# sydeng99/ssTEM-restoration

Hardware: AMD Instinct MI355X
Metric: restored megapixels/sec (interp+fusion fwd) at 1024x1024; PSNR vs ref (higher is better)
Workload: dtype f32; 1 GPU; SepConv 51-tap interpolation forward (pad + 2 sepconv + add + mean; one fused launch on the two gray planes, row-segment coefficients as the IFNet heads store them), batch=8 1024x1024 tiles per GPU; batch_per_gpu=8, taps=51, frame_planes=1, coefficient_layout=row-segments, compare_with_rounds_1_2=extra.apply_nchw_1024

## Files before the change

### sstem-restoration_amd/csrc/sepconv_kernels.hip

```cpp
#include <hip/hip_runtime.h>
#include <stdint.h>
#include <stdlib.h>

#include <atomic>
#include <mutex>
#include <unordered_map>

#include "sepconv_kernels.h"

#ifndef SSTEM_ABLATE
#define SSTEM_ABLATE 0
#endif
#ifndef SSTEM_HPF
#define SSTEM_HPF 11
#endif
#ifndef SSTEM_BLK_SKEWLD
#define SSTEM_BLK_SKEWLD 0
#endif
#ifndef SSTEM_GRAY_DMA
#define SSTEM_GRAY_DMA 1
#endif
#ifndef SSTEM_RGB_RING
#define SSTEM_RGB_RING 2
#endif
#ifndef SSTEM_GRAY16_ABLATE
#define SSTEM_GRAY16_ABLATE 0
#endif
#ifndef SSTEM_COEF_AUX
#define SSTEM_COEF_AUX 0
#endif
#ifndef SSTEM_PAIR_COEF_AUX
#define SSTEM_PAIR_COEF_AUX 2
#endif

namespace sstem {

constexpr int F = 51;
constexpr int KSTEPS = 54;
constexpr int TILE_COLS = 116;

__host__ __device__ constexpr int rm_pitch(int ch) { return ch == 2 ? 120 : 144; }
__host__ __device__ constexpr int rm_pitch_tile(int ch, int waves, int rpw)
{
    return (waves * rpw > 36) ? TILE_COLS : rm_pitch(ch);
}
static_assert((1 * rm_pitch(1) / 4) % 16 == 4 && (2 * rm_pitch(2) / 4) % 16 == 12 &&
              (3 * rm_pitch(3) / 4) % 16 == 12 && rm_pitch(2) >= TILE_COLS, "LDS row stride");

typedef float f32x4 __attribute__((ext_vector_type(4)));

template <bool BF> __device__ __forceinline__ float coef_at(const float* t, int64_t i)
{
    if constexpr (BF) return __builtin_bit_cast(float, (uint32_t)reinterpret_cast<const uint16_t*>(t)[i] << 16);
    else return t[i];
}
template <bool BF = false>
__global__ __launch_bounds__(256) void sepconv_fwd_direct(
    const float* __restrict__ in, const float* __restrict__ ver, const float* __restrict__ hor,
    float* __restrict__ out, int64_t B, int64_t C, int64_t H, int64_t W, int filt, const int* __restrict__ skip_if_gray = nullptr)
{
    if (skip_if_gray && *skip_if_gray != 0) return;
    const int64_t plane = H * W;
    const int64_t Hin = H + filt - 1, Win = W + filt - 1;
    const int64_t n = B * plane;
    for (int64_t p = (int64_t)blockIdx.x * blockDim.x + threadIdx.x; p < n;
         p += (int64_t)gridDim.x * blockDim.x) {
        const int64_t b = p / plane;
        const int64_t yx = p - b * plane;
        const int64_t y = yx / W, x = yx - y * W;
        const int64_t cbase = b * filt * plane + yx;
        for (int64_t c = 0; c < C; ++c) {
            const float* ip = in + ((b * C + c) * Hin + y) * Win + x;
            float acc = 0.f;
            for (int fy = 0; fy < filt; ++fy) {
                float t = 0.f;
                for (int fx = 0; fx < filt; ++fx)
                    t = fmaf(ip[(int64_t)fy * Win + fx], coef_at<BF>(hor, cbase + (int64_t)fx * plane), t);
                acc = fmaf(coef_at<BF>(ver, cbase + (int64_t)fy * plane), t, acc);
            }
            out[(b * C + c) * plane + yx] = acc;
        }
    }
}

template <bool VERTICAL, bool BF = false>
__global__ __launch_bounds__(256) void sepconv_grad_direct(
    const float* __restrict__ g, const float* __restrict__ in, const float* __restrict__ coef,
    float* __restrict__ gout, int64_t B, int64_t C, int64_t H, int64_t W, int filt, const int* __restrict__ skip_if_gray = nullptr)
{
    if (skip_if_gray && *skip_if_gray != 0) return;
    const int64_t plane = H * W;
    const int64_t Hin = H + filt - 1, Win = W + filt - 1;
    const int64_t n = B * filt * plane;
    for (int64_t p = (int64_t)blockIdx.x * blockDim.x + threadIdx.x; p < n;
         p += (int64_t)gridDim.x * blockDim.x) {
        const int64_t b = p / (filt * plane);
        const int64_t r = p - b * filt * plane;
        const int64_t f = r / plane;
        const int64_t yx = r - f * plane;
        const int64_t y = yx / W, x = yx - y * W;
        const int64_t cbase = b * filt * plane + yx;
        float acc = 0.f;
        for (int64_t c = 0; c < C; ++c) {
            const float gg = g[(b * C + c) * plane + yx];
            const float* ip = in + ((b * C + c) * Hin + y) * Win + x;
            float t = 0.f;
            if (VERTICAL) {
                for (int fx = 0; fx < filt; ++fx)
                    t = fmaf(ip[f * Win + fx], coef_at<BF>(coef, cbase + (int64_t)fx * plane), t);
            } else {
                for (int fy = 0; fy < filt; ++fy)
                    t = fmaf(ip[(int64_t)fy * Win + f], coef_at<BF>(coef, cbase + (int64_t)fy * plane), t);
            }
            acc = fmaf(gg, t, acc);
        }
        gout[p] = acc;
    }
}
// ... 785 lines not shown
                    const float res = ph ? (parked + csum) * (1.0f / 3) : csum;
                    *stg_ptr(dst, xoff) = res;
                    if (ph && fa.out_u8) fa.out_u8[(b * H + y) * W + x0 + lane] = numpy_u8_of(res);
                }
            }
            if constexpr (!PFH && BLK && SSTEM_BLK_SKEWLD) load_taps_skewed_buf(hc, rh, nextoff, pn, xoff, sub);
            else if constexpr (!PFH) load_taps_buf<BF>(hc, rh, nextoff, pn, xoff);
        };
        int nrows = 0;
        if (y0 + ywave < H) {
            const int64_t left = (H - 1 - (y0 + ywave)) / YSTEP + 1;
            nrows = left < RPW ? (int)left : RPW;
        }
        if constexpr (PFH) {
#pragma unroll 1
            for (int rr = 0; rr + 1 < nrows; rr += 2) {
                do_row(hs, hn, rr, true);
                do_row(hn, hs, rr + 1, rr + 2 < nrows);
            }
            if (nrows & 1) {
                do_row(hs, hn, nrows - 1, false);
                if (next_ph) {
#pragma unroll
                    for (int t = 0; t < KSTEPS; ++t) hs[t] = hn[t];
                }
            }
        } else {
            float dummy[1];
#pragma unroll 1
            for (int rr = 0; rr < nrows; ++rr) do_row(hs, dummy, rr, rr + 1 < nrows);
        }
    }
}

template <int I, int N, typename Fn>
__device__ __forceinline__ void static_for(Fn&& fn)
{
    if constexpr (I < N) {
        fn(std::integral_constant<int, I>{});
        static_for<I + 1, N>(fn);
    }
}

template <int WAVES, int RPW, int WPE>
__global__ __launch_bounds__(WAVES * 64, WPE) void sepconv_gray_mfma_pair(
    const float* __restrict__ in_a, const float* __restrict__ ver_a, const float* __restrict__ hor_a,
    float* __restrict__ out, TileArgs args, FusedArgs fa)
{
    static_assert(WAVES == 4, "the rows of a pair are one 4-row MFMA tile apart");
    static_assert(RPW % 2 == 0, "row pairs");
    if (fa.gray_flag && *fa.gray_flag == 0) return;
    constexpr int TR = WAVES * RPW;
    constexpr int ROWS = TR + F;
    constexpr int RS = rm_pitch(1);
    constexpr int YSTEP = WAVES;
    constexpr int NA = 2;
    constexpr int NGRP = 7;
    constexpr int LV = 2;
    constexpr uint32_t TAP = 256u;
    constexpr int AUX = SSTEM_PAIR_COEF_AUX;
    extern __shared__ __attribute__((aligned(16))) float lds[];

    int64_t b, ty, tx;
    decode_block(args, b, ty, tx);
    const int64_t H = args.H, W = args.W;
    const int64_t plane = H * W;
    const int wave = __builtin_amdgcn_readfirstlane(threadIdx.x >> 6);
    const int64_t y0 = ty * TR, x0 = tx * 64;

    const int lane = threadIdx.x & 63;
    const int blk = lane >> 2, sub = lane & 3;
    const bool xok = (x0 + lane) < W;
    const uint32_t xoff = (uint32_t)(xok ? lane : 0) * 4u;
    auto clampy = [&](int64_t y) __attribute__((always_inline)) -> int64_t { return y < H ? y : H - 1; };
    const int64_t yfirst = clampy(y0 + wave);

    const uint32_t seg_row = (uint32_t)args.tiles_x * (uint32_t)(F * 256);
    const uint32_t img_bytes = (uint32_t)H * seg_row;
    const int64_t img_elems = (int64_t)(img_bytes >> 2);
    const uint32_t seg_x = (uint32_t)tx * (uint32_t)(F * 256);
    auto rowoff = [&](int64_t y) __attribute__((always_inline)) -> uint32_t { return (uint32_t)clampy(y) * seg_row + seg_x; };

    float hA[KSTEPS], hB[KSTEPS], vA[F], vB[F];

    auto vload = [&](float (&v)[F], rsrc_t r, uint32_t ro, uint32_t ps, const int f0, const int f1) __attribute__((always_inline)) {
        uint32_t soff = ro + (uint32_t)f0 * ps;
        pin_s(soff);
#pragma unroll
        for (int f = 0; f < F; ++f) {
            if (f < f0 || f >= f1) continue;
            v[f] = bldc<false, AUX>(r, xoff, soff);
            soff += ps;
            pin_s(soff);
        }
    };
    auto vload_group = [&](const int k, rsrc_t r, uint32_t roA, uint32_t roB, uint32_t ps) __attribute__((always_inline)) {
        vload(vA, r, roA, ps, 8 * k, (8 * k + 8 < F) ? 8 * k + 8 : F);
        vload(vB, r, roB, ps, (8 * k - 4 > 0) ? 8 * k - 4 : 0, (8 * k + 4 < F) ? 8 * k + 4 : F);
    };
    auto hload = [&](float (&h)[KSTEPS], rsrc_t r, uint32_t ro, uint32_t ps, const int t0, const int t1) __attribute__((always_inline)) {
        if constexpr (SSTEM_BLK_SKEWLD) load_taps_skewed_buf<AUX>(h, r, ro, ps, xoff, sub, t0, t1 < KSTEPS ? t1 : KSTEPS);
        else load_taps_buf<false, AUX>(h, r, ro, ps, xoff, t0 < F ? t0 : F, t1 < F ? t1 : F);
    };
    {
        const rsrc_t rv = coef_rsrc_c<false>(ver_a, b * img_elems, img_bytes);
        const rsrc_t rh = coef_rsrc_c<false>(hor_a, b * img_elems, img_bytes);
        const uint32_t oA = rowoff(yfirst), oB = rowoff(yfirst + YSTEP);
#pragma unroll
        for (int k = 0; k < LV; ++k) vload_group(k, rv, oA, oB, TAP);
        hload(hA, rh, oA, TAP, 0, KSTEPS);
        hload(hB, rh, oB, TAP, 0, KSTEPS);
    }

#pragma unroll 1
    for (int ph = 0; ph < 2; ++ph) {
        const float* in = ph ? fa.in2 : in_a;
        const float* ver = ph ? fa.ver2 : ver_a;
        const float* hor = ph ? fa.hor2 : hor_a;
        const bool next_ph = ph == 0;
        const rsrc_t rv_cur = coef_rsrc_c<false>(ver, b * img_elems, img_bytes);
        const rsrc_t rh_cur = coef_rsrc_c<false>(hor, b * img_elems, img_bytes);
        const rsrc_t rv_nxt = coef_rsrc_c<false>(next_ph ? fa.ver2 : ver, b * img_elems, img_bytes);
        const rsrc_t rh_nxt = coef_rsrc_c<false>(next_ph ? fa.hor2 : hor, b * img_elems, img_bytes);

        if (ph) __syncthreads();
#if SSTEM_GRAY_DMA
        stage_gray_tile_dma<WAVES * 64, ROWS, RS, true>(lds, in + (b * args.in_planes) * plane, (int)H, (int)W, (int)y0, (int)x0);
#else
        stage_gray_tile<WAVES * 64, ROWS, RS, true>(lds, in + (b * args.in_planes) * plane, (int)H, (int)W, (int)y0, (int)x0);
#endif
        __syncthreads();

        int nrows = 0;
        if (y0 + wave < H) {
            const int64_t left = (H - 1 - (y0 + wave)) / YSTEP + 1;
            nrows = left < RPW ? (int)left : RPW;
        }
#pragma unroll 1
        for (int rr = 0; rr < nrows; rr += 2) {
            const bool more = rr + 2 < nrows;
            const bool two = rr + 1 < nrows;
            const int yl = wave + rr * YSTEP;
            const int64_t y = y0 + yl;
            const int64_t ynext = more ? (y + 2 * YSTEP) : (next_ph ? yfirst : y);
            const uint32_t pn = (more || next_ph) ? TAP : 0u;
            const uint32_t curA = rowoff(y), curB = rowoff(y + YSTEP);
            const uint32_t nxtA = rowoff(ynext), nxtB = rowoff(ynext + YSTEP);
            const rsrc_t rv_n = more ? rv_cur : rv_nxt;
            const rsrc_t rh_n = more ? rh_cur : rh_nxt;
            float* dstA = out + (b * H + y) * W + x0;
            float* dstB = out + (b * H + clampy(y + YSTEP)) * W + x0;
            pin_uniform(dstA);
            pin_uniform(dstB);
            const float parkedA = *stg_ptr(dstA, xoff);
            const float parkedB = *stg_ptr(dstB, xoff);

            if constexpr (!SSTEM_BLK_SKEWLD) {
                skew_taps_in_place(hA, sub);
                skew_taps_in_place(hB, sub);
            }
            const float* arow = lds + (yl + sub) * RS + blk * 4;
            f32x4 ar[2][NA];
#pragma unroll
            for (int c = 0; c < NA; ++c) ar[0][c] = *reinterpret_cast<const f32x4*>(arow + c * 4 * RS);
            float oA = 0.f, oB = 0.f;
            static_for<0, NGRP>([&](auto kc) __attribute__((always_inline)) {
                constexpr int k = decltype(kc)::value;
                if (k + LV < NGRP) vload_group(k + LV, rv_cur, curA, curB, TAP);
                else vload_group(k + LV - NGRP, rv_n, nxtA, nxtB, pn);
                f32x4 accA[NA], accB[NA];
#pragma unroll
                for (int c = 0; c < NA; ++c) { accA[c] = (f32x4){0.f, 0.f, 0.f, 0.f}; accB[c] = accA[c]; }
                const float* abase = arow + k * (NA * 4) * RS;
                const float* anext = arow + (k + 1) * (NA * 4) * RS;
#pragma unroll
                for (int tq = 0; tq < 14; ++tq) {
                    const int cc = k * 14 + tq;
                    if (tq + 1 < 14) {
#pragma unroll
                        for (int c = 0; c < NA; ++c)
                            ar[(cc + 1) % 2][c] = *reinterpret_cast<const f32x4*>(abase + c * 4 * RS + (tq + 1) * 4);
                    } else if (k + 1 < NGRP) {
#pragma unroll
                        for (int c = 0; c < NA; ++c)
                            ar[(cc + 1) % 2][c] = *reinterpret_cast<const f32x4*>(anext + c * 4 * RS);
                    }
                    __builtin_amdgcn_sched_barrier(0);
#pragma unroll
                    for (int e = 0; e < 4; ++e) {
                        const int t = tq * 4 + e;
                        if (t < KSTEPS) {
#pragma unroll
                            for (int c = 0; c < NA; ++c) {
                                const int a = 2 * k + c;
                                if (a <= 12) accA[c] = __builtin_amdgcn_mfma_f32_4x4x1f32(ar[cc % 2][c][e], hA[t], accA[c], 0, 0, 0);
                                if (a >= 1) accB[c] = __builtin_amdgcn_mfma_f32_4x4x1f32(ar[cc % 2][c][e], hB[t], accB[c], 0, 0, 0);
                            }
                        }
                    }
                    __builtin_amdgcn_sched_barrier(0);
                    if (k == NGRP - 1) {
                        hload(hA, rh_n, nxtA, pn, 4 * tq, 4 * tq + 4);
                        hload(hB, rh_n, nxtB, pn, 4 * tq, 4 * tq + 4);
                    }
                }
#pragma unroll
                for (int c = 0; c < NA; ++c) {
                    const int a = 2 * k + c;
                    if (a <= 12)
#pragma unroll
                        for (int i = 0; i < 4; ++i)
                            if (4 * a + i < F) oA = fmaf(vA[4 * a + i], accA[c][i], oA);
                }
#pragma unroll
                for (int c = 0; c < NA; ++c) {
                    const int a = 2 * k + c;
                    if (a >= 1)
#pragma unroll
                        for (int i = 0; i < 4; ++i)
                            if (4 * (a - 1) + i < F) oB = fmaf(vB[4 * (a - 1) + i], accB[c][i], oB);
                }
                asm volatile("" : "+v"(oA), "+v"(oB));
            });
            if (xok) {
                const float csA = (oA + oA) + oA;
                const float resA = ph ? (parkedA + csA) * (1.0f / 3) : csA;
                *stg_ptr(dstA, xoff) = resA;
                if (ph && fa.out_u8) fa.out_u8[(b * H + y) * W + x0 + lane] = numpy_u8_of(resA);
                if (two) {
                    const float csB = (oB + oB) + oB;
                    const float resB = ph ? (parkedB + csB) * (1.0f / 3) : csB;
                    *stg_ptr(dstB, xoff) = resB;
                    if (ph && fa.out_u8) fa.out_u8[(b * H + y + YSTEP) * W + x0 + lane] = numpy_u8_of(resB);
                }
            }
        }
    }
}

constexpr int G16_RS = 130;
template <int WAVES, int RPW, bool BLK, int VAR = 0>
__global__ __launch_bounds__(WAVES * 64, 2) void sepconv_gray16_mfma(
    const float* __restrict__ in_a, const float* __restrict__ ver_a, const float* __restrict__ hor_a,
    float* __restrict__ out, TileArgs args, FusedArgs fa)
{
    constexpr int TR = WAVES * RPW;
    constexpr int ROWS = TR + F;
    constexpr int RS = G16_RS;
    constexpr int IMG = ROWS * RS;
    extern __shared__ __attribute__((aligned(16))) float lds[];

    int64_t b, ty, tx;
    decode_block(args, b, ty, tx);
    const int64_t H = args.H, W = args.W;
    const int64_t plane = H * W;
    const int wave = __builtin_amdgcn_readfirstlane(threadIdx.x >> 6);
    const int64_t y0 = ty * TR, x0 = tx * 64;
    const int lane = threadIdx.x & 63;
    const int kq = lane >> 4, j = lane & 15;

    const uint32_t tap4 = BLK ? 256u : (uint32_t)plane * 4u;
    const uint32_t seg_row = (uint32_t)args.tiles_x * (uint32_t)(F * 256);
    const uint32_t img_bytes = BLK ? (uint32_t)H * seg_row : (uint32_t)F * tap4;
    const int64_t img_elems = BLK ? (int64_t)(img_bytes >> 2) : (int64_t)F * plane;
    const uint32_t seg_x = (uint32_t)tx * (uint32_t)(F * 256);
    auto rowoff = [&](int64_t y) __attribute__((always_inline)) -> uint32_t {
        return BLK ? (uint32_t)y * seg_row + seg_x : (uint32_t)(y * W + x0) * 4u;
    };
    const rsrc_t rv0 = coef_rsrc(ver_a + b * img_elems, img_bytes), rh0 = coef_rsrc(hor_a + b * img_elems, img_bytes);
    const rsrc_t rv1 = coef_rsrc(fa.ver2 + b * img_elems, img_bytes), rh1 = coef_rsrc(fa.hor2 + b * img_elems, img_bytes);

    const int d = kq - j;
    const int c = d & 3, sh = -(d >> 2);
    const bool s1 = sh & 1, s2 = sh & 2, s4 = sh & 4, c3 = c == 3;
    const uint32_t vh = (uint32_t)c * tap4 + (uint32_t)j * 4u;
    const uint32_t vv = (uint32_t)(4 * kq) * tap4 + (uint32_t)j * 4u;
    const uint32_t vr = (uint32_t)j * 4u;

    float Bh[4][17], Vv[4][15];
    auto request = [&](const int cg0, const int NC, const rsrc_t rh, const rsrc_t rv, const uint32_t off) __attribute__((always_inline)) {
        uint32_t so = off;
        pin_s(so);
#pragma unroll
        for (int n = 0; n < 13; ++n) {
#pragma unroll
            for (int q = 0; q < NC; ++q) Bh[cg0 + q][n] = bld(rh, vh + (uint32_t)(cg0 + q) * 64u, so);
            so += 4u * tap4;
            pin_s(so);
        }
#pragma unroll
        for (int T = 0; T < 3; ++T) {
            so = off + (uint32_t)(16 * T) * tap4;
            pin_s(so);
#pragma unroll
            for (int r = 0; r < 4; ++r) {
#pragma unroll
                for (int q = 0; q < NC; ++q) Vv[cg0 + q][4 * T + r] = bld(rv, vv + (uint32_t)(cg0 + q) * 64u, so);
                so += tap4;
                pin_s(so);
            }
        }
        so = off + 48u * tap4;
        pin_s(so);
#pragma unroll
        for (int r = 0; r < 3; ++r) {
#pragma unroll
            for (int q = 0; q < NC; ++q) Vv[cg0 + q][12 + r] = bld(rv, vr + (uint32_t)(cg0 + q) * 64u, so);
            so += tap4;
            pin_s(so);
        }
    };

    int nrows = 0;
    if (y0 + wave < H) {
        const int64_t left = (H - 1 - (y0 + wave)) / WAVES + 1;
        nrows = left < RPW ? (int)left : RPW;
    }
    if (nrows > 0) {
        const uint32_t off = rowoff(y0 + wave);
        request(0, 2, rh0, rv0, off);
// ... 1339 lines not shown
                                 const TileArgs& a, hipStream_t s, const int* flag = nullptr)
{
    return gradh_coalesce() ? launch_gradh_vc<CH, WAVES, RPW, true>(in, g, ver, gh, a, s, flag)
                            : launch_gradh_vc<CH, WAVES, RPW, false>(in, g, ver, gh, a, s, flag);
}

static hipError_t launch_rgb_gradh_stream(const float* in, const float* g, const float* ver, float* gh, TileArgs a, hipStream_t s,
                                          const int* flag)
{
    constexpr int WAVES = 8, RPW = 4, TR = WAVES * RPW;
    constexpr int ROWS = TR + F + 4;
    constexpr int PITCH_T = ((ROWS + 3) / 4 * 4) | 4;
    constexpr size_t lds_bytes = (size_t)3 * TCOLS * PITCH_T * sizeof(float);
    static_assert(lds_bytes <= 160 * 1024, "LDS");
    auto k = sepconv_rgb_gradh_stream_mfma<WAVES, RPW>;
    static std::atomic<uint64_t> lds_set{0};
    const hipError_t attr = set_lds(k, lds_bytes, lds_set);
    if (attr != hipSuccess) return attr;
    a.tiles_y = (a.H + TR - 1) / TR;
    const int64_t nwg = a.B * a.tiles_y * a.tiles_x;
    if (nwg <= 0 || nwg > 0x7fffffffLL) return hipErrorInvalidValue;
    hipLaunchKernelGGL(k, dim3((unsigned)nwg), dim3(WAVES * 64), lds_bytes, s, in, g, ver, gh, a, flag);
    return hipGetLastError();
}

template <int CH>
static hipError_t launch_gradh(const float* in, const float* g, const float* ver, float* gh,
                               const TileArgs& a, hipStream_t s)
{
    switch (tile_variant()) {
        case 1: return launch_gradh_v<CH, 12, 3>(in, g, ver, gh, a, s);
        case 2: return launch_gradh_v<CH, 12, 2>(in, g, ver, gh, a, s);
        case 3: return launch_gradh_v<CH, 16, 2>(in, g, ver, gh, a, s);
        case 4: return launch_gradh_v<CH, 16, 3>(in, g, ver, gh, a, s);
        default: return launch_gradh_v<CH, 8, 4>(in, g, ver, gh, a, s);
    }
}

static TileArgs make_args(int64_t B, int64_t C, int64_t H, int64_t W)
{
    TileArgs a;
    a.B = B; a.C = C; a.H = H; a.W = W;
    a.tiles_x = (W + 63) / 64;
    const int tr = tile_rows(tile_variant());
    a.tiles_y = (H + tr - 1) / tr;
    a.c0 = 0;
    a.in_planes = 3;
    static const int dbg = [] { const char* d = getenv("SSTEM_DEBUG_FLAGS"); return d ? atoi(d) : 0; }();
    a.dbg = dbg;
    return a;
}

bool mfma_grid_ok(int64_t B, int64_t H, int64_t W)
{
    TileArgs a = make_args(B, 1, H, W);
    const int64_t nwg = a.B * a.tiles_y * a.tiles_x;
    return nwg > 0 && nwg <= 0x7fffffffLL;
}

template <int MODE, int WAVES, int RPW, int WPE, bool PFH, int RING, bool BLK = false, bool BF = false>
static hipError_t launch_gray_v(const float* in, const float* ver, const float* hor, float* out, TileArgs a,
                                hipStream_t s, const FusedArgs& fa)
{
    constexpr int TR = WAVES * RPW;
    constexpr size_t lds_bytes = (size_t)(TR + F) * rm_pitch(1) * sizeof(float);
    static_assert(lds_bytes <= 160 * 1024, "LDS");
    auto k = sepconv_gray_mfma<MODE, WAVES, RPW, WPE, PFH, RING, BLK, BF>;
    static std::atomic<uint64_t> lds_set{0};
    const hipError_t attr = set_lds(k, lds_bytes, lds_set);
    if (attr != hipSuccess) return attr;
    a.tiles_y = (a.H + TR - 1) / TR;
    const int64_t nwg = a.B * a.tiles_y * a.tiles_x;
    if (nwg <= 0 || nwg > 0x7fffffffLL) return hipErrorInvalidValue;
    hipLaunchKernelGGL(k, dim3((unsigned)nwg), dim3(WAVES * 64), lds_bytes, s, in, ver, hor, out, a, fa);
    return hipGetLastError();
}

static int gray_pair_variant()
{
    static const int v = [] { const char* e = getenv("SSTEM_GRAY_PAIR"); return e ? atoi(e) : 1; }();
    return v;
}

template <int WAVES, int RPW, int WPE>
static hipError_t launch_gray_pair_v(const float* in, const float* ver, const float* hor, float* out, TileArgs a,
                                     hipStream_t s, const FusedArgs& fa)
{
    constexpr int TR = WAVES * RPW;
    constexpr size_t lds_bytes = (size_t)(TR + F) * rm_pitch(1) * sizeof(float);
    static_assert(lds_bytes * WPE <= 160 * 1024, "LDS");
    auto k = sepconv_gray_mfma_pair<WAVES, RPW, WPE>;
    static std::atomic<uint64_t> lds_set{0};
    const hipError_t attr = set_lds(k, lds_bytes, lds_set);
    if (attr != hipSuccess) return attr;
    a.tiles_y = (a.H + TR - 1) / TR;
    const int64_t nwg = a.B * a.tiles_y * a.tiles_x;
    if (nwg <= 0 || nwg > 0x7fffffffLL) return hipErrorInvalidValue;
    hipLaunchKernelGGL(k, dim3((unsigned)nwg), dim3(WAVES * 64), lds_bytes, s, in, ver, hor, out, a, fa);
    return hipGetLastError();
}

template <int MODE, bool BLK = false>
static hipError_t launch_gray(const float* in, const float* vg, const float* hor, float* out, TileArgs a,
                              hipStream_t s, const FusedArgs& fa)
{
    static const int forced = [] { const char* e = getenv("SSTEM_GRAY_SHAPE"); return e ? atoi(e) : -1; }();
    const int pair = gray_pair_variant();
    (void)pair;
    int shape = forced;
    if (shape < 0) {
        shape = (a.B * a.tiles_x * ((a.H + 63) / 64) >= 1024) ? 3 : 0;
        if (shape == 0 && a.B * a.tiles_x * ((a.H + 31) / 32) < 512) shape = 7;
    }
    if (BLK && forced < 0 && shape == 3) shape = 0;
    if constexpr (BLK) {
        switch (shape) {
            case 3: return launch_gray_v<MODE, 4, 16, 2, true, 2, true>(in, vg, hor, out, a, s, fa);
            case 7: return launch_gray_v<MODE, 4, 4, 3, false, 2, true>(in, vg, hor, out, a, s, fa);
            default:
                if constexpr (MODE == 2) {
                    const bool two_per_cu = a.B * a.tiles_x * ((a.H + 63) / 64) >= 512;
                    if (pair == 2 || (pair == 1 && two_per_cu)) return launch_gray_pair_v<4, 16, 2>(in, vg, hor, out, a, s, fa);
                }
                return launch_gray_v<MODE, 4, 8, 3, false, 2, true>(in, vg, hor, out, a, s, fa);
        }
    }
    switch (shape) {
        case 1: return launch_gray_v<MODE, 4, 8, 2, true, 3>(in, vg, hor, out, a, s, fa);
        case 2: return launch_gray_v<MODE, 4, 16, 2, true, 3>(in, vg, hor, out, a, s, fa);
        case 3: return launch_gray_v<MODE, 4, 16, 2, true, 2>(in, vg, hor, out, a, s, fa);
        case 4: return launch_gray_v<MODE, 4, 8, 2, false, 3>(in, vg, hor, out, a, s, fa);
        case 5: return launch_gray_v<MODE, 4, 16, 2, false, 3>(in, vg, hor, out, a, s, fa);
        case 6: return launch_gray_v<MODE, 2, 8, 3, false, 2>(in, vg, hor, out, a, s, fa);
        case 7: return launch_gray_v<MODE, 4, 4, 3, false, 2>(in, vg, hor, out, a, s, fa);
        case 8: return launch_gray_v<MODE, 2, 4, 3, false, 2>(in, vg, hor, out, a, s, fa);
        default: return launch_gray_v<MODE, 4, 8, 3, false, 2>(in, vg, hor, out, a, s, fa);
    }
}

static bool rgb_stream_enabled(int64_t H, int64_t W)
{
    static const bool on = [] { const char* e = getenv("SSTEM_RGB_STREAM"); return !(e && atoi(e) == 0); }();
    return on && (uint64_t)F * (uint64_t)H * (uint64_t)W * 4u < (1ull << 32) && (uint64_t)3 * (uint64_t)(H + F) * (uint64_t)(W + F) * 4u < (1ull << 32);
}

template <int MODE>
static hipError_t launch_rgb_stream(const float* in, const float* ver, const float* hor, float* out, TileArgs a, hipStream_t s,
                                    const FusedArgs& fa)
{
    constexpr int WAVES = 8, RPW = 4, TR = WAVES * RPW;
    constexpr size_t lds_bytes = (size_t)(TR + F) * 3 * rm_pitch(3) * sizeof(float);
    static_assert(lds_bytes <= 160 * 1024, "LDS");
    auto k = sepconv_rgb_stream_mfma<MODE, WAVES, RPW>;
    static std::atomic<uint64_t> lds_set{0};
    const hipError_t attr = set_lds(k, lds_bytes, lds_set);
    if (attr != hipSuccess) return attr;
    a.tiles_y = (a.H + TR - 1) / TR;
    const int64_t nwg = a.B * a.tiles_y * a.tiles_x;
    if (nwg <= 0 || nwg > 0x7fffffffLL) return hipErrorInvalidValue;
    hipLaunchKernelGGL(k, dim3((unsigned)nwg), dim3(WAVES * 64), lds_bytes, s, in, ver, hor, out, a, fa);
    return hipGetLastError();
}

static bool gray_dispatch_enabled(int64_t H, int64_t W)
{
    static const bool on = [] { const char* e = getenv("SSTEM_GRAY_KERNEL"); return !(e && atoi(e) == 0); }();
    return on && (uint64_t)F * (uint64_t)H * (uint64_t)W * 4u < (1ull << 32);
}

hipError_t launch_fwd_mfma(const float* in, const float* ver, const float* hor, float* out,
                           int64_t B, int64_t C, int64_t H, int64_t W, hipStream_t s)
{
    TileArgs a = make_args(B, C, H, W);
    hipError_t e = hipSuccess;
    int* flag = nullptr;
    if (C == 3 && gray_dispatch_enabled(H, W) && tile_rows(tile_variant()) == 32) {
        flag = next_gray_flag(s, e);
        if (e != hipSuccess) return e;
    }
    if (flag) {
        e = launch_detect(in, nullptr, B, (H + F - 1) * (W + F - 1), flag, s);
        if (e != hipSuccess) return e;
        const FusedArgs fa{nullptr, nullptr, nullptr, flag};
        if (rgb_stream_enabled(H, W)) e = launch_rgb_stream<0>(in, ver, hor, out, a, s, fa);
        else switch (tile_variant()) {
            case 0: e = launch_rowmajor_v<0, 3, 8, 4>(in, ver, hor, out, a, s, fa); break;
            default: e = launch_rowmajor_v<0, 3, 16, 2>(in, ver, hor, out, a, s, fa); break;
        }
        if (e != hipSuccess) return e;
        return launch_gray<0>(in, ver, hor, out, a, s, fa);
    }
    if (C == 3 && rgb_stream_enabled(H, W))
        return launch_rgb_stream<0>(in, ver, hor, out, a, s, FusedArgs{nullptr, nullptr, nullptr, nullptr});
    for (int64_t c0 = 0; c0 < C && e == hipSuccess; c0 += 3) {
        a.c0 = (int)c0;
        const int64_t ch = (C - c0) < 3 ? (C - c0) : 3;
        if (ch == 3) e = launch_rowmajor<0, 3>(in, ver, hor, out, a, s);
        else if (ch == 2) e = launch_rowmajor<0, 2>(in, ver, hor, out, a, s);
        else e = launch_rowmajor<0, 1>(in, ver, hor, out, a, s);
    }
    return e;
}

hipError_t launch_interp_fused(const float* i1, const float* i2, const float* k1v, const float* k1h,
                               const float* k2v, const float* k2h, float* out, int64_t B, int64_t H, int64_t W,
// ... 250 lines not shown
    else e = launch_rowmajor<1, 1>(in, g, hor, gv, a, s);
    if (e != hipSuccess) return e;
    if (C == 3 && rgb_stream_enabled(H, W) && gradh_coalesce()) e = launch_rgb_gradh_stream(in, g, ver, gh, a, s, nullptr);
    else if (C == 3) e = launch_gradh<3>(in, g, ver, gh, a, s);
    else if (C == 2) e = launch_gradh<2>(in, g, ver, gh, a, s);
    else e = launch_gradh<1>(in, g, ver, gh, a, s);
    return e;
}

static bool gray_bf16_ok(int64_t C, int64_t H, int64_t W)
{
    return C == 3 && gray_dispatch_enabled(H, W) && tile_rows(tile_variant()) == 32;
}

hipError_t launch_fwd_bf16coef(const float* in, const uint16_t* ver, const uint16_t* hor, float* out,
                               int64_t B, int64_t C, int64_t H, int64_t W, hipStream_t s)
{
    const float* v = reinterpret_cast<const float*>(ver);
    const float* h = reinterpret_cast<const float*>(hor);
    hipError_t e = hipSuccess;
    int* flag = nullptr;
    if (gray_bf16_ok(C, H, W)) {
        flag = next_gray_flag(s, e);
        if (e != hipSuccess) return e;
    }
    if (flag) {
        e = launch_detect(in, nullptr, B, (H + F - 1) * (W + F - 1), flag, s);
        if (e != hipSuccess) return e;
    }
    hipLaunchKernelGGL(sepconv_fwd_direct<true>, dim3(grid_1d(B * H * W, 256)), dim3(256), 0, s, in, v, h, out, B, C, H, W, F, (const int*)flag);
    e = hipGetLastError();
    if (e != hipSuccess || !flag) return e;
    TileArgs a = make_args(B, C, H, W);
    const FusedArgs fa{nullptr, nullptr, nullptr, flag};
    if (a.B * a.tiles_x * ((a.H + 31) / 32) < 512) return launch_gray_v<0, 4, 4, 3, false, 2, false, true>(in, v, h, out, a, s, fa);
    return launch_gray_v<0, 4, 8, 3, false, 2, false, true>(in, v, h, out, a, s, fa);
}

hipError_t launch_bwd_bf16coef(const float* g, const float* in, const uint16_t* ver, const uint16_t* hor,
                               float* gv, float* gh, int64_t B, int64_t C, int64_t H, int64_t W, hipStream_t s)
{
    const float* v = reinterpret_cast<const float*>(ver);
    const float* h = reinterpret_cast<const float*>(hor);
    hipError_t e = hipSuccess;
    int* flag = nullptr;
    if (gray_bf16_ok(C, H, W)) {
        flag = next_gray_flag(s, e);
        if (e != hipSuccess) return e;
    }
    if (flag) {
        e = launch_detect(in, nullptr, B, (H + F - 1) * (W + F - 1), flag, s);
        if (e != hipSuccess) return e;
    }
    const int grid = grid_1d(B * F * H * W, 256);
    hipLaunchKernelGGL((sepconv_grad_direct<true, true>), dim3(grid), dim3(256), 0, s, g, in, h, gv, B, C, H, W, F, (const int*)flag);
    e = hipGetLastError();
    if (e != hipSuccess) return e;
    hipLaunchKernelGGL((sepconv_grad_direct<false, true>), dim3(grid), dim3(256), 0, s, g, in, v, gh, B, C, H, W, F, (const int*)flag);
    e = hipGetLastError();
    if (e != hipSuccess || !flag) return e;
    TileArgs a = make_args(B, C, H, W);
    e = launch_gray_gradv_v<4, 8, 3, false, 2, true>(in, g, h, gv, a, s, flag);
    if (e != hipSuccess) return e;
    return launch_gray_gradh_v<4, 8, 3, false, 2, true, true>(in, g, v, gh, a, s, flag);
}

bool interp_fused_gray_bf16coef_ok(int64_t H, int64_t W) { return interp_fused_gray_ok(H, W); }

hipError_t launch_interp_fused_gray_bf16coef(const float* g1, const float* g2, const uint16_t* k1v, const uint16_t* k1h,
                                             const uint16_t* k2v, const uint16_t* k2h, float* out, int64_t B, int64_t H, int64_t W,
                                             hipStream_t s)
{
    if (!interp_fused_gray_bf16coef_ok(H, W)) return hipErrorInvalidValue;
    TileArgs a = make_args(B, 3, H, W);
    a.in_planes = 1;
    const FusedArgs fa{g1, reinterpret_cast<const float*>(k1v), reinterpret_cast<const float*>(k1h), nullptr};
    const float* v2 = reinterpret_cast<const float*>(k2v);
    const float* h2 = reinterpret_cast<const float*>(k2h);
    if (a.B * a.tiles_x * ((a.H + 31) / 32) < 512) return launch_gray_v<2, 4, 4, 3, false, 2, false, true>(g2, v2, h2, out, a, s, fa);
    return launch_gray_v<2, 4, 8, 3, false, 2, false, true>(g2, v2, h2, out, a, s, fa);
}

}
```

Baseline: 6499 megapixels/s.

## Add software-pipelined pair kernel with uneven tap-group split and interleaved loads

Measured after the change: 6586 megapixels/s, median of 6. 1.01x the previous value.

```diff
diff --git a/sstem-restoration_amd/csrc/sepconv_kernels.hip b/sstem-restoration_amd/csrc/sepconv_kernels.hip
--- a/sstem-restoration_amd/csrc/sepconv_kernels.hip
+++ b/sstem-restoration_amd/csrc/sepconv_kernels.hip
@@ -32,8 +32,48 @@
 #ifndef SSTEM_PAIR_COEF_AUX
 #define SSTEM_PAIR_COEF_AUX 2
 #endif
+#ifndef SSTEM_HP_T0
+#define SSTEM_HP_T0 4
+#define SSTEM_HP_T1 4
+#define SSTEM_HP_T2 2
+#endif
+#ifndef SSTEM_HP_VEARLY
+#define SSTEM_HP_VEARLY 16
+#endif
+#ifndef SSTEM_HP_PHASE_CT
+#define SSTEM_HP_PHASE_CT 1
+#endif
+#ifndef SSTEM_PAIR_STAMP
+#define SSTEM_PAIR_STAMP 0
+#endif
 
 namespace sstem {
+
+#if SSTEM_PAIR_STAMP
+constexpr int PAIR_STAMP_WGS = 2048;
+constexpr int PAIR_STAMP_PER_WG = 2 * 8 * 5;
+__device__ unsigned long long g_pair_stamps[PAIR_STAMP_WGS * PAIR_STAMP_PER_WG];
+#endif
+__device__ __forceinline__ bool pair_stamp_on(int wave)
+{
+#if SSTEM_PAIR_STAMP
+    return wave == 0 && blockIdx.x < (unsigned)PAIR_STAMP_WGS;
+#else
+    return false;
+#endif
+}
+template <int P>
+__device__ __forceinline__ void pair_stamp(bool on, int ph, int pair)
+{
+#if SSTEM_PAIR_STAMP
+    __builtin_amdgcn_sched_barrier(0);
+    if (on) {
+        const unsigned long long t = __builtin_amdgcn_s_memtime();
+        if ((threadIdx.x & 63) == 0) g_pair_stamps[(size_t)blockIdx.x * PAIR_STAMP_PER_WG + (ph * 8 + pair) * 5 + P] = t;
+    }
+    __builtin_amdgcn_sched_barrier(0);
+#endif
+}
 
 constexpr int F = 51;
 constexpr int KSTEPS = 54;
@@ -985,6 +1025,7 @@
     auto rowoff = [&](int64_t y) __attribute__((always_inline)) -> uint32_t { return (uint32_t)clampy(y) * seg_row + seg_x; };
 
     float hA[KSTEPS], hB[KSTEPS], vA[F], vB[F];
+    const bool stamp = pair_stamp_on(wave);
 
     auto vload = [&](float (&v)[F], rsrc_t r, uint32_t ro, uint32_t ps, const int f0, const int f1) __attribute__((always_inline)) {
         uint32_t soff = ro + (uint32_t)f0 * ps;
@@ -1055,6 +1096,7 @@
             float* dstB = out + (b * H + clampy(y + YSTEP)) * W + x0;
             pin_uniform(dstA);
             pin_uniform(dstB);
+            pair_stamp<0>(stamp, ph, rr >> 1);
             const float parkedA = *stg_ptr(dstA, xoff);
             const float parkedB = *stg_ptr(dstB, xoff);
 
@@ -1062,6 +1104,7 @@
                 skew_taps_in_place(hA, sub);
                 skew_taps_in_place(hB, sub);
             }
+            pair_stamp<1>(stamp, ph, rr >> 1);
             const float* arow = lds + (yl + sub) * RS + blk * 4;
             f32x4 ar[2][NA];
 #pragma unroll
@@ -1069,6 +1112,8 @@
             float oA = 0.f, oB = 0.f;
             static_for<0, NGRP>([&](auto kc) __attribute__((always_inline)) {
                 constexpr int k = decltype(kc)::value;
+                if constexpr (k == 1) pair_stamp<2>(stamp, ph, rr >> 1);
+                if constexpr (k == NGRP - 1) pair_stamp<3>(stamp, ph, rr >> 1);
                 if (k + LV < NGRP) vload_group(k + LV, rv_cur, curA, curB, TAP);
                 else vload_group(k + LV - NGRP, rv_n, nxtA, nxtB, pn);
                 f32x4 accA[NA], accB[NA];
@@ -1137,8 +1182,257 @@
                     if (ph && fa.out_u8) fa.out_u8[(b * H + y + YSTEP) * W + x0 + lane] = numpy_u8_of(resB);
                 }
             }
-        }
-    }
+            pair_stamp<4>(stamp, ph, rr >> 1);
+        }
+    }
+}
+constexpr int HP_NP = (SSTEM_HP_T0 + SSTEM_HP_T1 + SSTEM_HP_T2 < 14) ? 4 : 3;
+constexpr int hp_a0(int h)
+{
+    return h <= 0 ? 0 : (h == 1 ? SSTEM_HP_T0 : (h == 2 ? SSTEM_HP_T0 + SSTEM_HP_T1 : (h < HP_NP ? SSTEM_HP_T0 + SSTEM_HP_T1 + SSTEM_HP_T2 : 14)));
+}
+constexpr int hp_nt(int h) { return hp_a0(h + 1) - hp_a0(h); }
+constexpr int hp_min(int a, int b) { return a < b ? a : b; }
+constexpr int hp_max(int a, int b) { return a > b ? a : b; }
+constexpr int hp_fa0(int h) { return 4 * hp_a0(h); }
+constexpr int hp_fa1(int h) { return hp_min(4 * hp_a0(h + 1), F); }
+constexpr int hp_fb0(int h) { return 4 * hp_max(hp_a0(h) - 1, 0); }
+constexpr int hp_fb1(int h) { return hp_min(4 * (hp_a0(h + 1) - 1), F); }
+constexpr int hp_nv(int h) { return (hp_fa1(h) - hp_fa0(h)) + (hp_fb1(h) - hp_fb0(h)); }
+constexpr int HP_NV = hp_max(hp_max(hp_nv(0), hp_nv(1)), hp_max(hp_nv(2), hp_nv(3)));
+constexpr int hp_vbase(int h) { return h <= 0 ? 0 : (hp_vbase(h - 1) + hp_nv(h - 1)) % HP_NV; }
+constexpr int hp_vearly(int h) { return (h >= 1 && h < HP_NP) ? hp_min(hp_min(hp_nv(h), HP_NV - hp_nv(h - 1)), SSTEM_HP_VEARLY) : 0; }
+constexpr int HP_EPC = 4;
+constexpr int hp_vpc(int h) { return h == HP_NP - 1 ? 6 : 8; }
+constexpr int hp_vown_chunks(int h) { return (hp_nv(h) - hp_vearly(h) + hp_vpc(h) - 1) / hp_vpc(h); }
+constexpr int hp_read_off(int s, int rs)
+{
+    int h = 0;
+    while (h + 1 < HP_NP && s >= 14 * hp_a0(h + 1)) ++h;
+    const int i = s - 14 * hp_a0(h);
+    return (hp_a0(h) + i % hp_nt(h)) * 4 * rs + (i / hp_nt(h)) * 4;
+}
+constexpr bool hp_split_ok()
+{
+    for (int h = 0; h < HP_NP; ++h)
+        if (hp_nt(h) <= 0 || hp_nt(h) % 2 != 0 || hp_vown_chunks(h) * HP_EPC + hp_vearly(h + 1) > 14 * HP_EPC) return false;
+    return hp_a0(HP_NP) == 14 && hp_a0(HP_NP - 1) < 14;
+}
+static_assert(hp_split_ok(), "tile split");
+
+template <int WAVES, int RPW, int WPE>
+__global__ __launch_bounds__(WAVES * 64, WPE) void sepconv_gray_mfma_pair_hp(
+    const float* __restrict__ in_a, const float* __restrict__ ver_a, const float* __restrict__ hor_a,
+    float* __restrict__ out, TileArgs args, FusedArgs fa)
+{
+    static_assert(WAVES == 4, "the rows of a pair are one 4-row MFMA tile apart");
+    static_assert(RPW % 2 == 0, "row pairs");
+    if (fa.gray_flag && *fa.gray_flag == 0) return;
+    constexpr int TR = WAVES * RPW;
+    constexpr int ROWS = TR + F;
+    constexpr int RS = rm_pitch(1);
+    constexpr int YSTEP = WAVES;
+    constexpr int NRD = 14 * 14;
+    constexpr int RING = 2;
+    constexpr uint32_t TAP = 256u;
+    constexpr int AUX = SSTEM_PAIR_COEF_AUX;
+    extern __shared__ __attribute__((aligned(16))) float lds[];
+
+    int64_t b, ty, tx;
+    decode_block(args, b, ty, tx);
+    const int64_t H = args.H, W = args.W;
+    const int64_t plane = H * W;
+    const int wave = __builtin_amdgcn_readfirstlane(threadIdx.x >> 6);
+    const int64_t y0 = ty * TR, x0 = tx * 64;
+
+    const int lane = threadIdx.x & 63;
+    const int blk = lane >> 2, sub = lane & 3;
+    const bool xok = (x0 + lane) < W;
+    const uint32_t xoff = (uint32_t)(xok ? lane : 0) * 4u;
+    auto clampy = [&](int64_t y) __attribute__((always_inline)) -> int64_t { return y < H ? y : H - 1; };
+    const int64_t yfirst = clampy(y0 + wave);
+
+    const uint32_t seg_row = (uint32_t)args.tiles_x * (uint32_t)(F * 256);
+    const uint32_t img_bytes = (uint32_t)H * seg_row;
+    const int64_t img_elems = (int64_t)(img_bytes >> 2);
+    const uint32_t seg_x = (uint32_t)tx * (uint32_t)(F * 256);
+    auto rowoff = [&](int64_t y) __attribute__((always_inline)) -> uint32_t { return (uint32_t)clampy(y) * seg_row + seg_x; };
+    const bool m1 = sub >= 1, m2 = sub >= 2, m3 = sub == 3;
+    const bool stamp = pair_stamp_on(wave);
+    const rsrc_t rout = __builtin_amdgcn_make_buffer_rsrc(out + b * plane, 0, (int)((uint32_t)plane * 4u), 0x00020000);
+    const rsrc_t rout8 = __builtin_amdgcn_make_buffer_rsrc(fa.out_u8 ? fa.out_u8 + b * plane : nullptr, 0, fa.out_u8 ? (int)(uint32_t)plane : 0, 0x00020000);
+
+    float hA[KSTEPS], hB[KSTEPS], v[HP_NV];
+
+    auto vreq = [&](auto hc, rsrc_t r, uint32_t roA, uint32_t roB, const int i0, const int i1) __attribute__((always_inline)) {
+        constexpr int h = decltype(hc)::value;
+        constexpr int nA = hp_fa1(h) - hp_fa0(h), n = hp_nv(h), vb = hp_vbase(h);
+        uint32_t so = roA + (uint32_t)(hp_fa0(h) + i0) * TAP;
+        pin_s(so);
+#pragma unroll
+        for (int i = 0; i < HP_NV; ++i) {
+            if (i < i0 || i >= i1 || i >= nA) continue;
+            v[(vb + i) % HP_NV] = bldc<false, AUX>(r, xoff, so);
+            so += TAP;
+            pin_s(so);
+        }
+        so = roB + (uint32_t)(hp_fb0(h) + (i0 > nA ? i0 - nA : 0)) * TAP;
+        pin_s(so);
+#pragma unroll
+        for (int i = 0; i < HP_NV; ++i) {
+            if (i < i0 || i >= i1 || i < nA || i >= n) continue;
+            v[(vb + i) % HP_NV] = bldc<false, AUX>(r, xoff, so);
+            so += TAP;
+            pin_s(so);
+        }
+    };
+    auto hload = [&](float (&h)[KSTEPS], rsrc_t r, uint32_t ro, uint32_t ps, const int t0, const int t1) __attribute__((always_inline)) {
+        load_taps_buf<false, AUX>(h, r, ro, ps, xoff, t0 < F ? t0 : F, t1 < F ? t1 : F);
+    };
+    {
+        const rsrc_t rh = coef_rsrc_c<false>(hor_a, b * img_elems, img_bytes);
+        hload(hA, rh, rowoff(yfirst), TAP, 0, KSTEPS);
+        hload(hB, rh, rowoff(yfirst + YSTEP), TAP, 0, KSTEPS);
+    }
+
+    auto phase = [&](auto phc) __attribute__((always_inline)) {
+        const int ph = phc;
+        const float* in = ph ? fa.in2 : in_a;
+        const float* ver = ph ? fa.ver2 : ver_a;
+        const float* hor = ph ? fa.hor2 : hor_a;
+        const bool next_ph = ph == 0;
+        const rsrc_t rv_cur = coef_rsrc_c<false>(ver, b * img_elems, img_bytes);
+        const rsrc_t rh_cur = coef_rsrc_c<false>(hor, b * img_elems, img_bytes);
+        const rsrc_t rh_nxt = coef_rsrc_c<false>(next_ph ? fa.hor2 : hor, b * img_elems, img_bytes);
+
+        if (ph) __syncthreads();
+        stage_gray_tile_dma<WAVES * 64, ROWS, RS, true>(lds, in + (b * args.in_planes) * plane, (int)H, (int)W, (int)y0, (int)x0);
+        __syncthreads();
+
+        int nrows = 0;
+        if (y0 + wave < H) {
+            const int64_t left = (H - 1 - (y0 + wave)) / YSTEP + 1;
+            nrows = left < RPW ? (int)left : RPW;
+        }
+#pragma unroll 1
+        for (int rr = 0; rr < nrows; rr += 2) {
+            const bool more = rr + 2 < nrows;
+            const bool two = rr + 1 < nrows;
+            const int yl = wave + rr * YSTEP;
+            const int64_t y = y0 + yl;
+            const int64_t ynext = more ? (y + 2 * YSTEP) : (next_ph ? yfirst : y);
+            const uint32_t pn = (more || next_ph) ? TAP : 0u;
+            const uint32_t curA = rowoff(y), curB = rowoff(y + YSTEP);
+            const uint32_t nxtA = rowoff(ynext), nxtB = rowoff(ynext + YSTEP);
+            const rsrc_t rh_n = more ? rh_cur : rh_nxt;
+            uint32_t dstA = (uint32_t)(y * W + x0) * 4u;
+            uint32_t dstB = (uint32_t)(clampy(y + YSTEP) * W + x0) * 4u;
+            pin_s(dstA);
+            pin_s(dstB);
+            pair_stamp<0>(stamp, ph, rr >> 1);
+            float parkedA = 0.f, parkedB = 0.f;
+            if (ph) {
+                parkedA = bld<0>(rout, xoff, dstA);
+                parkedB = bld<0>(rout, xoff, dstB);
+            }
+            const float* arow = lds + (yl + sub) * RS + blk * 4;
+            f32x4 ar[RING][2];
+#pragma unroll
+            for (int d = 0; d < 2; ++d) ar[0][d] = *reinterpret_cast<const f32x4*>(arow + hp_read_off(d, RS));
+            float oA = 0.f, oB = 0.f;
+            float cA0 = 0.f, cA1 = 0.f, cA2 = 0.f, cB0 = 0.f, cB1 = 0.f, cB2 = 0.f;
+            static_for<0, HP_NP>([&](auto hc) __attribute__((always_inline)) {
+                constexpr int h = decltype(hc)::value;
+                constexpr int NT = hp_nt(h), A0 = hp_a0(h), VPC = hp_vpc(h), E = hp_vearly(h), CO = hp_vown_chunks(h), VB = hp_vbase(h);
+                if constexpr (h == 1) pair_stamp<2>(stamp, ph, rr >> 1);
+                if constexpr (h == HP_NP - 1) pair_stamp<3>(stamp, ph, rr >> 1);
+                f32x4 accA[NT], accB[NT];
+#pragma unroll
+                for (int c = 0; c < NT; ++c) { accA[c] = (f32x4){0.f, 0.f, 0.f, 0.f}; accB[c] = accA[c]; }
+                static_for<0, 14>([&](auto qc) __attribute__((always_inline)) {
+                    constexpr int q = decltype(qc)::value;
+                    if constexpr (q < CO) vreq(hc, rv_cur, curA, curB, E + VPC * q, E + VPC * q + VPC);
+                    else if constexpr (HP_EPC * (q - CO) < hp_vearly(h + 1))
+                        vreq(std::integral_constant<int, h + 1>{}, rv_cur, curA, curB, HP_EPC * (q - CO), hp_min(HP_EPC * (q - CO) + HP_EPC, hp_vearly(h + 1)));
+                    if constexpr (h == 0) {
+#pragma unroll
+                        for (int e = 0; e < 4; ++e) {
+                            const int t = 4 * q + e;
+                            if (t < KSTEPS) {
+                                const float rA = (t < F) ? hA[t] : 0.f, rB = (t < F) ? hB[t] : 0.f;
+                                hA[t] = m3 ? cA0 : (m2 ? cA1 : (m1 ? cA2 : rA));
+                                hB[t] = m3 ? cB0 : (m2 ? cB1 : (m1 ? cB2 : rB));
+                                cA0 = cA1; cA1 = cA2; cA2 = rA;
+                                cB0 = cB1; cB1 = cB2; cB2 = rB;
+                            }
+                        }
+                        if constexpr (q == 0) pair_stamp<1>(stamp, ph, rr >> 1);
+                    }
+#pragma unroll
+                    for (int c = 0; c < NT; c += 2) {
+                        const int s = 14 * A0 + q * NT + c;
+                        if (s + 2 < NRD) {
+#pragma unroll
+                            for (int d = 0; d < 2; ++d)
+                                ar[(s / 2 + 1) % RING][d] = *reinterpret_cast<const f32x4*>(arow + hp_read_off(s + 2 + d, RS));
+                        }
+                        __builtin_amdgcn_sched_barrier(0);
+#pragma unroll
+                        for (int e = 0; e < 4; ++e) {
+                            const int t = 4 * q + e;
+                            if (t < KSTEPS) {
+#pragma unroll
+                                for (int d = 0; d < 2; ++d) {
+                                    const int a = A0 + c + d;
+                                    if (a <= 12) accA[c + d] = __builtin_amdgcn_mfma_f32_4x4x1f32(ar[(s / 2) % RING][d][e], hA[t], accA[c + d], 0, 0, 0);
+                                    if (a >= 1) accB[c + d] = __builtin_amdgcn_mfma_f32_4x4x1f32(ar[(s / 2) % RING][d][e], hB[t], accB[c + d], 0, 0, 0);
+                                }
+                            }
+                        }
+                        __builtin_amdgcn_sched_barrier(0);
+                    }
+                    if constexpr (h == HP_NP - 1) {
+                        hload(hA, rh_n, nxtA, pn, 4 * q, 4 * q + 4);
+                        hload(hB, rh_n, nxtB, pn, 4 * q, 4 * q + 4);
+                    }
+                });
+                {
+                    constexpr int fa0 = hp_fa0(h), fb0 = hp_fb0(h), nA = hp_fa1(h) - hp_fa0(h);
+#pragma unroll
+                    for (int c = 0; c < NT; ++c)
+#pragma unroll
+                        for (int i = 0; i < 4; ++i)
+                            if (A0 + c <= 12 && 4 * (A0 + c) + i < F) oA = fmaf(v[(VB + 4 * (A0 + c) + i - fa0) % HP_NV], accA[c][i], oA);
+#pragma unroll
+                    for (int c = 0; c < NT; ++c)
+#pragma unroll
+                        for (int i = 0; i < 4; ++i)
+                            if (A0 + c >= 1 && 4 * (A0 + c - 1) + i < F) oB = fmaf(v[(VB + nA + 4 * (A0 + c - 1) + i - fb0) % HP_NV], accB[c][i], oB);
+                }
+                asm volatile("" : "+v"(oA), "+v"(oB));
+            });
+            if (xok) {
+                const float csA = (oA + oA) + oA;
+                const float resA = ph ? (parkedA + csA) * (1.0f / 3) : csA;
+                __builtin_amdgcn_raw_buffer_store_b32(__builtin_bit_cast(int, resA), rout, (int)xoff, (int)dstA, 0);
+                if (ph && fa.out_u8) __builtin_amdgcn_raw_buffer_store_b8(numpy_u8_of(resA), rout8, (int)(xoff >> 2), (int)(dstA >> 2), 0);
+                if (two) {
+                    const float csB = (oB + oB) + oB;
+                    const float resB = ph ? (parkedB + csB) * (1.0f / 3) : csB;
+                    __builtin_amdgcn_raw_buffer_store_b32(__builtin_bit_cast(int, resB), rout, (int)xoff, (int)dstB, 0);
+                    if (ph && fa.out_u8) __builtin_amdgcn_raw_buffer_store_b8(numpy_u8_of(resB), rout8, (int)(xoff >> 2), (int)(dstB >> 2), 0);
+                }
+            }
+            pair_stamp<4>(stamp, ph, rr >> 1);
+        }
+    };
+#if SSTEM_HP_PHASE_CT
+    phase(std::integral_constant<int, 0>{});
+    phase(std::integral_constant<int, 1>{});
+#else
+#pragma unroll 1
+    for (int ph = 0; ph < 2; ++ph) phase(ph);
+#endif
 }
 
 constexpr int G16_RS = 130;
@@ -2644,14 +2938,14 @@
     return v;
 }
 
-template <int WAVES, int RPW, int WPE>
+template <int WAVES, int RPW, int WPE, bool HP = false>
 static hipError_t launch_gray_pair_v(const float* in, const float* ver, const float* hor, float* out, TileArgs a,
                                      hipStream_t s, const FusedArgs& fa)
 {
     constexpr int TR = WAVES * RPW;
     constexpr size_t lds_bytes = (size_t)(TR + F) * rm_pitch(1) * sizeof(float);
     static_assert(lds_bytes * WPE <= 160 * 1024, "LDS");
-    auto k = sepconv_gray_mfma_pair<WAVES, RPW, WPE>;
+    auto k = HP ? sepconv_gray_mfma_pair_hp<WAVES, RPW, WPE> : sepconv_gray_mfma_pair<WAVES, RPW, WPE>;
     static std::atomic<uint64_t> lds_set{0};
     const hipError_t attr = set_lds(k, lds_bytes, lds_set);
     if (attr != hipSuccess) return attr;
@@ -2682,7 +2976,8 @@
             default:
                 if constexpr (MODE == 2) {
                     const bool two_per_cu = a.B * a.tiles_x * ((a.H + 63) / 64) >= 512;
-                    if (pair == 2 || (pair == 1 && two_per_cu)) return launch_gray_pair_v<4, 16, 2>(in, vg, hor, out, a, s, fa);
+                    if (pair == 3 || (pair == 1 && two_per_cu)) return launch_gray_pair_v<4, 16, 2, true>(in, vg, hor, out, a, s, fa);
+                    if (pair == 2) return launch_gray_pair_v<4, 16, 2>(in, vg, hor, out, a, s, fa);
                 }
                 return launch_gray_v<MODE, 4, 8, 3, false, 2, true>(in, vg, hor, out, a, s, fa);
         }
@@ -3099,3 +3394,13 @@
 }
 
 }
+
+#if SSTEM_PAIR_STAMP
+extern "C" int sstem_debug_pair_stamps(unsigned long long* out, long long n)
+{
+    const size_t total = (size_t)sstem::PAIR_STAMP_WGS * sstem::PAIR_STAMP_PER_WG;
+    if (n < 0 || (size_t)n > total) return -1;
+    if (hipDeviceSynchronize() != hipSuccess) return -1;
+    return hipMemcpyFromSymbol(out, HIP_SYMBOL(sstem::g_pair_stamps), (size_t)n * sizeof(unsigned long long)) == hipSuccess ? 0 : -1;
+}
+#endif
```
